# OpenRendererBenchmark/libYafaRay

Hardware: AMD Instinct MI355X
Metric: Mrays/sec (primary+secondary) on the path-tracing hot path (higher is better)
Workload: dtype f32; 1 GPU; 1M-tri diffuse Cornell-box soup 512x512 64spp primary+1-bounce (BASELINE.json metric config); triangles=1000000, width=512, height=512, spp=64, bounces=1, lights=1, parallelism=pixel-tile shard x1, film_reduce=none, kd_nodes=2803313, kd_leaf_refs=3155999, kd_max_depth=27

## Files before the change

### include/yafgpu.h

```cpp
#ifndef YAFGPU_H
#define YAFGPU_H

#include <stdint.h>

#ifdef __cplusplus
extern "C" {
#endif

#define YAFGPU_FILM_CHANNELS 5
#define YAFGPU_FILM_PLANES   4

enum { YAFGPU_MAT_SHINYDIFFUSE = 0, YAFGPU_MAT_GLOSSY = 1, YAFGPU_MAT_LIGHT = 2, YAFGPU_MAT_GLASS = 3, YAFGPU_MAT_MIRROR = 4,
       YAFGPU_MAT_COATED_GLOSSY = 5,
       YAFGPU_MAT_ROUGH_GLASS = 6,
       YAFGPU_MAT_MASKED = 7,
       YAFGPU_MAT_BLEND = 8 };
enum { YAFGPU_LIGHT_AREA = 0, YAFGPU_LIGHT_POINT = 1, YAFGPU_LIGHT_DIRECTIONAL = 2, YAFGPU_LIGHT_SUN = 3, YAFGPU_LIGHT_SPHERE = 4,
       YAFGPU_LIGHT_BACKGROUND = 5,
       YAFGPU_LIGHT_MESH = 7,
       YAFGPU_LIGHT_PORTAL = 8,
       YAFGPU_LIGHT_IES = 9, YAFGPU_LIGHT_IES_SOFT = 10,
       YAFGPU_LIGHT_SPOT = 11, YAFGPU_LIGHT_SPOT_SOFT = 12 };
enum { YAFGPU_BACKGROUND_NONE = 0, YAFGPU_BACKGROUND_CONSTANT = 1, YAFGPU_BACKGROUND_TEXTURE = 2,
       YAFGPU_BACKGROUND_GRADIENT = 4, YAFGPU_BACKGROUND_SUNSKY = 5 };
// ... 309 lines not shown
	int32_t format;
	int32_t image_width, image_height, border_x, border_y;
} yafgpu_image_desc;
uint64_t yafgpu_image_bytes(int32_t format, int32_t width, int32_t height);
int yafgpu_film_to_image(const float *d_film, const yafgpu_image_desc *desc, void *d_image, void *stream);
int yafgpu_scene_film_to_image(yafgpu_scene_t *scene, const yafgpu_image_desc *desc, void *h_image);

int yafgpu_render_passes_to_host(yafgpu_scene_t *scene, const yafgpu_render_params *rp, const yafgpu_aa_schedule *aa,
                                 float *h_film, yafgpu_counters *h_counters, int32_t *resampled);
int yafgpu_render_to_host(yafgpu_scene_t *scene, const yafgpu_render_params *rp, float *h_film, yafgpu_counters *h_counters);

int yafgpu_trace_closest(yafgpu_scene_t *scene, int32_t n, const float *rays, int32_t *tri, float *t, float *bary);
int yafgpu_trace_shadow(yafgpu_scene_t *scene, int32_t n, const float *rays, int32_t *shadowed);
uint32_t yafgpu_trace_reservation(uint32_t n, uint32_t seen, uint32_t waves);
void yafgpu_trace_schedule(uint32_t info[8]);

int yafgpu_set_profiling(yafgpu_scene_t *scene, int32_t enable);
int yafgpu_scene_set_pass_pipelining(yafgpu_scene_t *scene, int32_t mode);
void yafgpu_glibc_rand(uint32_t seed, int32_t count, int32_t *out);
int yafgpu_scene_set_abort_flag(yafgpu_scene_t *scene, const volatile int32_t *flag);
typedef int (*yafgpu_exchange_fn)(void *user, float *d_values, uint64_t n_floats);
int yafgpu_scene_set_exchange(yafgpu_scene_t *scene, yafgpu_exchange_fn fn, void *user);
int yafgpu_get_profile(const yafgpu_scene_t *scene, double ms[4], uint64_t launches[4]);

int yafgpu_probe(yafgpu_scene_t *scene, int32_t op, int32_t n, const float *in, int32_t n_in, float *out, int32_t n_out);

typedef struct yafgpu_kdtree yafgpu_kdtree_t;
yafgpu_kdtree_t *yafgpu_kdtree_build_device(const float *verts, int32_t n_tris);
yafgpu_kdtree_t *yafgpu_kdtree_build(const float *verts, int32_t n_tris, int32_t threads);
void yafgpu_kdtree_info(const yafgpu_kdtree_t *tree, yafgpu_tree_info *info);
void yafgpu_kdtree_get(const yafgpu_kdtree_t *tree, uint32_t *nodes, uint32_t *refs, float bound6[6]);
int32_t yafgpu_kdtree_treelets(const uint32_t *nodes, uint32_t n_nodes, int32_t inline_leaves, uint32_t *words, uint32_t *n_words,
                               uint32_t *leaves, uint32_t *n_leaves, uint32_t *root);
void yafgpu_kdtree_destroy(yafgpu_kdtree_t *tree);

int yafgpu_scene_get_tree(const yafgpu_scene_t *scene, uint32_t *nodes, uint32_t *refs, float bound6[6]);

#ifdef __cplusplus
}
#endif
#endif
```

### libyafaray_amd/csrc/kdtree_build.cpp

```cpp
#include "kdtree_build.h"

#include <algorithm>
#include <chrono>
#include <cmath>
#include <cstdlib>
#include <cstring>
#include <future>
#include <thread>
#include <utility>

namespace yafgpu {
namespace {

struct Box { float lo[3], hi[3]; };

struct Params
{
	const Box *prim_box;
	const float *verts;
	int depth_cap;
	float cost_ratio, empty_bonus;
};

struct Sub
// ... 326 lines not shown
		todo.emplace_back(g, (uint32_t)t);
		return (uint32_t)t << 2;
	};
	out.root = link_of(0u);
	while(!todo.empty() && !overflow)
	{
		const auto [g, t] = todo.back(); todo.pop_back();
		uint32_t w[8] = {nodes[g].a, 0u, 0u, nodes[g].b & 3u, 0u, 0u, 0u, 0u};
		const uint32_t child[2] = {g + 1u, nodes[g].b >> 2};
		uint32_t grand[4] = {0u, 0u, 0u, 0u}; bool interior[2];
		for(int k = 0; k < 2; ++k)
		{
			const KdNode &c = nodes[child[k]];
			interior[k] = (c.b & 3u) != 3u;
			w[1 + k] = interior[k] ? c.a : 0u;
			w[3] |= (interior[k] ? (c.b & 3u) : 3u) << (2 * (k + 1));
			if(interior[k]) { grand[2 * k] = child[k] + 1u; grand[2 * k + 1] = c.b >> 2; }
		}
		uint32_t links[4] = {0u, 0u, 0u, 0u};
		const size_t mark = todo.size();
		for(int k = 0; k < 2; ++k)
		{
			if(!interior[k]) { links[2 * k] = leaf_link(nodes[child[k]]); continue; }
			links[2 * k] = link_of(grand[2 * k]);
			links[2 * k + 1] = link_of(grand[2 * k + 1]);
		}
		std::reverse(todo.begin() + (std::ptrdiff_t)mark, todo.end());
		for(int k = 0; k < 4; ++k) w[4 + k] = links[k];
		std::memcpy(&out.words[(size_t)t * 8], w, sizeof w);
	}
	return overflow ? -2 : 0;
}

}

#include "../../include/yafgpu.h"
struct yafgpu_kdtree { yafgpu::KdTree t; int n_tris; };
extern "C" {
int32_t yafgpu_kdtree_treelets(const uint32_t *nodes, uint32_t n_nodes, int32_t inline_leaves, uint32_t *words, uint32_t *n_words,
                                uint32_t *leaves, uint32_t *n_leaves, uint32_t *root)
{
	std::vector<yafgpu::KdNode> tn(n_nodes);
	if(n_nodes) std::memcpy(tn.data(), nodes, (size_t)n_nodes * sizeof(yafgpu::KdNode));
	yafgpu::TreeletLayout tl;
	if(const int rc = yafgpu::build_treelets(tn, inline_leaves != 0, tl)) return rc;
	if(words && tl.words.size() <= *n_words && !tl.words.empty()) std::memcpy(words, tl.words.data(), tl.words.size() * 4);
	if(leaves && tl.leaves.size() <= *n_leaves && !tl.leaves.empty()) std::memcpy(leaves, tl.leaves.data(), tl.leaves.size() * 4);
	*n_words = (uint32_t)tl.words.size(); *n_leaves = (uint32_t)tl.leaves.size(); *root = tl.root;
	return 0;
}
yafgpu_kdtree_t *yafgpu_kdtree_build(const float *verts, int32_t n_tris, int32_t threads)
{
	auto *k = new yafgpu_kdtree();
	k->n_tris = n_tris;
	yafgpu::build_kdtree(verts, n_tris, 48, threads, k->t);
	return k;
}
void yafgpu_internal_set_error(const char *msg);
yafgpu_kdtree_t *yafgpu_kdtree_build_device(const float *verts, int32_t n_tris)
{
	auto *k = new yafgpu_kdtree();
	k->n_tris = n_tris;
	std::string err;
	if(yafgpu::build_kdtree_device_retry(verts, n_tris, 48, k->t, &err)) { yafgpu_internal_set_error(err.c_str()); delete k; return nullptr; }
	return k;
}
void yafgpu_kdtree_info(const yafgpu_kdtree_t *k, yafgpu_tree_info *info)
{
	info->n_nodes = (uint32_t)k->t.nodes.size(); info->n_leaf_refs = (uint32_t)k->t.refs.size();
	info->max_depth = (uint32_t)k->t.max_depth; info->n_tris = (uint32_t)k->n_tris;
	info->build_seconds = k->t.build_seconds; info->upload_seconds = 0; info->device_bytes = 0;
}
void yafgpu_kdtree_get(const yafgpu_kdtree_t *k, uint32_t *nodes, uint32_t *refs, float bound6[6])
{
	if(nodes && !k->t.nodes.empty()) std::memcpy(nodes, k->t.nodes.data(), k->t.nodes.size() * sizeof(yafgpu::KdNode));
	if(refs && !k->t.refs.empty()) std::memcpy(refs, k->t.refs.data(), k->t.refs.size() * sizeof(uint32_t));
	if(bound6) for(int i = 0; i < 3; ++i) { bound6[i] = k->t.bound_lo[i]; bound6[3 + i] = k->t.bound_hi[i]; }
}
void yafgpu_kdtree_destroy(yafgpu_kdtree_t *k) { delete k; }
}
```

### libyafaray_amd/csrc/kdtree_build.h

```cpp
#pragma once
#include <cstdint>
#include <string>
#include <vector>

namespace yafgpu {

struct KdNode { uint32_t a, b; };

struct KdTree
{
	std::vector<KdNode> nodes;
	std::vector<uint32_t> refs;
	float bound_lo[3], bound_hi[3];
	int max_depth = 0;
	double build_seconds = 0;
};

void build_kdtree(const float *verts, int n_tris, int depth_cap, int threads, KdTree &out);

int build_kdtree_device(const float *verts, int n_tris, int depth_cap, KdTree &out, std::string *err, int room = 1);
int build_kdtree_device_retry(const float *verts, int n_tris, int depth_cap, KdTree &out, std::string *err);

constexpr uint32_t kLinkLeaf = 0x80000000u, kLinkEscape = 0x40000000u, kLinkIndex = 0x3fffffffu, kLinkEmpty = kLinkLeaf;
constexpr uint32_t kLinkFirstBits = 24u, kLinkCountMax = 63u;
struct TreeletLayout
{
	std::vector<uint32_t> words;
	std::vector<uint32_t> leaves;
	uint32_t root = kLinkEmpty;
};
int build_treelets(const std::vector<KdNode> &nodes, bool inline_leaves, TreeletLayout &out);

}
```

### libyafaray_amd/csrc/yafgpu_device.hip

```cpp
#include <hip/hip_runtime.h>

#include <algorithm>
#include <atomic>
#include <chrono>
#include <cmath>
#include <cstdio>
#include <cstdlib>
#include <cstring>
#include <string>
#include <vector>
#include <map>
#include <memory>
#include <mutex>

#include "../../include/yafgpu.h"
#include "kdtree_build.h"
#include "yafgpu_math.h"
#include "yafgpu_shading.h"
#include "yafgpu_texture.h"
#include "yafgpu_assemble.h"

namespace yafgpu {

constexpr int kWave = 64;
constexpr int kBlock = 256;
constexpr int kWavesPerBlock = kBlock / kWave;
#ifndef YAFGPU_STACK
#define YAFGPU_STACK 8
#endif
constexpr int kStack = YAFGPU_STACK;
constexpr int kDepthCap = 48;
constexpr float kMinRayDist = (float)0.00005;
constexpr float kShadowBias = (float)0.0005;

struct DevScene
{
	const uint2 *nodes;
	const uint4 *treelets;
	const uint2 *tl_leaves;
	uint32_t tl_root;
	const uint32_t *refs;
	const float4 *tri;
	const float4 *tri_ng;
	const float4 *tri_vn;
	const yafgpu_material *mats;
	const yafgpu_light *lights;
	const int *faure;
	const int *faure_far;
	const int *faure_off;
	const double *inv_prims;
	int n_lights, n_tris, n_mats, n_faure;
	int faure_near;
	uint32_t n_nodes;
	float blo[3], bhi[3];
	yafgpu_camera cam;
	TexScene tex;
	BgScene bg;
	const float *lgeo;
};

struct RenderArgs
{
	DevScene sc;
	yafgpu_render_params rp;
	float shadow_bias, ray_min_dist, filterw;
	float table_scale; int wide_filter;
	const float *filter_table;
	int n_tiles;
	const int4 *tile_rect;
	float *planes;
	yafgpu_counters *counters;
};

struct LaneCounters { uint32_t closest, shadow, interior, leaves, tests, samples, restarts; };

// ... 832 lines not shown
	if(!bg_has_energy(row[1])) bad |= 1u << 16;
	row[kBgFlag] = __uint_as_float(bad);
}

YG_DEV void lgeo_rows(yafgpu_light *lights, int k, float *lgeo)
{
	const int n = lights[k].mesh_count;
	float *row = lgeo + lights[k].mesh_row, *func = row + kLgeoFunc;
	for(int i = (int)threadIdx.x; i < n; i += (int)blockDim.x)
	{
		const float *q = lgeo + 9 * (size_t)(lights[k].mesh_pool + i);
		const V3 a = vec3(q), edge_1 = vec3(q + 3) - a, edge_2 = vec3(q + 6) - a;
		func[i] = (float)(0.5 * (double)length(cross(edge_1, edge_2)));
	}
	__syncthreads();
	if(threadIdx.x != 0) return;
	double total_area = 0.0;
	for(int i = 0; i < n; ++i) total_area += (double)func[i];
	const float integral = pdf1d_cumulate(func, n, func + n);
	row[0] = integral; row[1] = 1.f / integral;
	lights[k].area = (float)total_area;
}
__global__ __launch_bounds__(kBlock) void meshlight_rows_kernel(yafgpu_light *lights, int n_lights, float *lgeo)
{
	const int k = (int)blockIdx.x;
	if(k >= n_lights || lights[k].type != YAFGPU_LIGHT_MESH) return;
	lgeo_rows(lights, k, lgeo);
}
__global__ __launch_bounds__(kBlock) void portallight_rows_kernel(yafgpu_light *lights, int n_lights, float *lgeo)
{
	const int k = (int)blockIdx.x;
	if(k >= n_lights || lights[k].type != YAFGPU_LIGHT_PORTAL) return;
	lgeo_rows(lights, k, lgeo);
}

}

using namespace yafgpu;

static float host_fsin(float x);
static thread_local std::string g_err;
static int fail(int code, const std::string &msg) { g_err = msg; return code; }
#define HIP_OK(expr) do { hipError_t e_ = (expr); if(e_ != hipSuccess) return fail(-100, std::string(#expr) + ": " + hipGetErrorString(e_)); } while(0)

template<typename T> struct DevMem
{
	T *p = nullptr; size_t cap = 0;
	DevMem() = default;
	DevMem(const DevMem &) = delete; DevMem &operator=(const DevMem &) = delete;
	~DevMem() { if(p) (void)hipFree(p); }
	hipError_t alloc(size_t count) { return hipMalloc((void **)&p, std::max<size_t>(count, 1) * sizeof(T)); }
	hipError_t reserve(size_t count, hipStream_t stream)
	{
		if(p && count <= cap) return hipSuccess;
		hipError_t e = hipStreamSynchronize(stream);
		if(e != hipSuccess) return e;
		if(p) (void)hipFree(p);
		p = nullptr; cap = 0;
		if((e = alloc(count)) != hipSuccess) { p = nullptr; return e; }
		cap = count;
		return hipSuccess;
	}
	operator T *() const { return p; }
};
struct Stream
{
// ... 553 lines not shown
	if(on_device)
	{
		std::string err;
		const int brc = build_kdtree_device_retry(rows.verts, n_tris, kDepthCap, s->tree, &err);
		if(brc == -2 || brc == -3) build_kdtree(rows.verts, n_tris, kDepthCap, d->build_threads, s->tree);
		else if(brc) return fail(-20, err);
	}
	else build_kdtree(rows.verts, n_tris, kDepthCap, d->build_threads, s->tree);
	s->info.build_seconds = s->tree.build_seconds;
	s->info.n_nodes = (uint32_t)s->tree.nodes.size();
	s->info.n_leaf_refs = (uint32_t)s->tree.refs.size();
	s->info.max_depth = (uint32_t)s->tree.max_depth;
	s->info.n_tris = (uint32_t)n_tris;
	return 0;
}

static int upload_tree(yafgpu_scene *s)
{
	DevScene &dv = s->dev;
	int rc = 0;
	if((rc = upload(s, (const uint2 *)s->tree.nodes.data(), s->tree.nodes.size(), &dv.nodes))) return rc;
	const char *e = std::getenv("YAFGPU_TREELET_INLINE");
	TreeletLayout tl;
	if(build_treelets(s->tree.nodes, !(e && std::atoi(e) == 0), tl)) return fail(-2, "kd-tree too large for the treelet layout");
	dv.tl_root = tl.root;
	if((rc = upload(s, (const uint4 *)tl.words.data(), tl.words.size() / 4, &dv.treelets))) return rc;
	if((rc = upload(s, (const uint2 *)tl.leaves.data(), tl.leaves.size() / 2, &dv.tl_leaves))) return rc;
	if((rc = upload(s, s->tree.refs.data(), s->tree.refs.size(), &dv.refs))) return rc;
	dv.n_nodes = (uint32_t)s->tree.nodes.size();
	for(int k = 0; k < 3; ++k) { dv.blo[k] = s->tree.bound_lo[k]; dv.bhi[k] = s->tree.bound_hi[k]; }
	return 0;
}

static int upload_lights(yafgpu_scene *s, const yafgpu_scene_desc *d)
{
	s->h_lights.assign(d->lights, d->lights + d->n_lights);
	bool with_tris = false;
	for(const yafgpu_light &l : s->h_lights) with_tris = with_tris || l.type == YAFGPU_LIGHT_MESH || l.type == YAFGPU_LIGHT_PORTAL;
	size_t row = with_tris ? (size_t)std::max(d->n_light_tris, 0) * 9 : 0;
	for(yafgpu_light &l : s->h_lights)
		if(l.type == YAFGPU_LIGHT_MESH || l.type == YAFGPU_LIGHT_PORTAL) { l.mesh_row = (int32_t)row; row += 2 * (size_t)l.mesh_count + 3; }
	row = (row + 3) & ~(size_t)3;
	for(yafgpu_light &l : s->h_lights)
		if(l.type == YAFGPU_LIGHT_PORTAL) { l.mesh_first = row <= (size_t)INT32_MAX ? (int32_t)row : 0; row += 16 * (size_t)l.mesh_count; }
	s->ies_base = row;
	for(const yafgpu_light &l : s->h_lights) s->has_ies = s->has_ies || l.type == YAFGPU_LIGHT_IES || l.type == YAFGPU_LIGHT_IES_SOFT;
	if(s->has_ies) row += (size_t)d->n_ies_floats;
	for(yafgpu_light &l : s->h_lights)
		if(l.type == YAFGPU_LIGHT_IES || l.type == YAFGPU_LIGHT_IES_SOFT) l.ies_first = row <= (size_t)INT32_MAX ? (int32_t)(s->ies_base + (size_t)l.ies_first) : 0;
	if(row > (size_t)INT32_MAX) return fail(-3, "the light-geometry pool outgrows 2^31 floats");
	s->lgeo_floats = row;
	const int rc = upload(s, s->h_lights.data(), s->h_lights.size(), &s->dev.lights);
	if(rc) return rc;
	s->dev.n_lights = s->n_lights = d->n_lights;
	for(const yafgpu_light &l : s->h_lights) s->light_mask |= 1u << (uint32_t)l.type;
	if(d->background.kind == YAFGPU_BACKGROUND_TEXTURE) s->light_mask |= 1u << (uint32_t)YAFGPU_LIGHT_BACKGROUND;
	return 0;
}

static int upload_textures(yafgpu_scene *s, const yafgpu_scene_desc *d)
{
	DevScene &dv = s->dev;
	std::memset(&dv.tex, 0, sizeof dv.tex);
	if(!((d->n_nodes > 0 && d->nodes) || d->background.kind == YAFGPU_BACKGROUND_TEXTURE)) return 0;
	int rc = 0;
	const float4 *texels = nullptr;
// ... 141 lines not shown

const char *yafgpu_last_error(void) { return g_err.c_str(); }
extern "C" void yafgpu_internal_set_error(const char *msg) { g_err = msg ? msg : ""; }

int yafgpu_device_count(void)
{
	int n = 0;
	if(hipGetDeviceCount(&n) != hipSuccess) return 0;
	return n;
}
int yafgpu_set_device(int device) { HIP_OK(hipSetDevice(device)); return 0; }

uint64_t yafgpu_planes_bytes(int32_t width, int32_t height)
{
	return (uint64_t)YAFGPU_FILM_PLANES * (uint64_t)width * (uint64_t)height * YAFGPU_FILM_CHANNELS * sizeof(float);
}

int yafgpu_scene_create(const yafgpu_scene_desc *d, yafgpu_scene_t **out)
{
	if(!out) return fail(-1, "null argument");
	int rc = check_desc(d);
	if(rc) return rc;
	std::unique_ptr<yafgpu_scene> owner(new yafgpu_scene());
	yafgpu_scene *s = owner.get();
	classify_materials(s, d);
	AssembledRows rows;
	const auto tr = std::chrono::steady_clock::now();
	if(d->inst.n_segments <= 0) host_rows(d, rows);
	else if((rc = assemble_scene(s, d, rows))) return rc;
	const double rows_seconds = std::chrono::duration<double>(std::chrono::steady_clock::now() - tr).count();
	if((rc = build_tree(s, d, rows))) return rc;
	const auto t1 = std::chrono::steady_clock::now();
	DevScene &dv = s->dev;
	if((rc = upload_tree(s)) || (rc = upload_rows(s, d, rows))) return rc;
	dv.tri = rows.rec; dv.tri_ng = rows.ng; dv.tri_vn = rows.vn; dv.mats = rows.mats;
	dv.n_tris = (int)rows.n; dv.n_mats = d->n_materials;
	if((rc = upload_lights(s, d)) || (rc = upload_textures(s, d)) || (rc = upload_nodes(s, d, rows)) || (rc = upload_qmc_tables(s))) return rc;
	dv.cam = d->camera;
	bokeh_table(dv.cam);
	s->mats.assign(d->materials, d->materials + d->n_materials);
	if((rc = background_tables(s, d)) || (rc = mesh_light_rows(s, d))) return rc;
	s->info.upload_seconds = std::chrono::duration<double>(std::chrono::steady_clock::now() - t1).count() + rows_seconds;
	*out = owner.release();
	return 0;
}

void yafgpu_scene_destroy(yafgpu_scene_t *s) { delete s; }

int yafgpu_scene_info(const yafgpu_scene_t *s, yafgpu_tree_info *info)
{
	if(!s || !info) return fail(-1, "null argument");
	*info = s->info;
	return 0;
}

int yafgpu_scene_get_tree(const yafgpu_scene_t *s, uint32_t *nodes, uint32_t *refs, float bound6[6])
{
	if(!s) return fail(-1, "null argument");
	if(nodes) std::memcpy(nodes, s->tree.nodes.data(), s->tree.nodes.size() * sizeof(KdNode));
	if(refs) std::memcpy(refs, s->tree.refs.data(), s->tree.refs.size() * sizeof(uint32_t));
	if(bound6) for(int k = 0; k < 3; ++k) { bound6[k] = s->tree.bound_lo[k]; bound6[3 + k] = s->tree.bound_hi[k]; }
	return 0;
}

static float host_fexp2(float x)
{
	x = std::min(x, 129.00000f);
// ... 1299 lines not shown
```

### libyafaray_amd/csrc/yafgpu_wavefront.h

```cpp
#pragma once

#include <stdint.h>
#if defined(__HIPCC__)
#define YAFGPU_HOST_DEVICE __host__ __device__
#else
#define YAFGPU_HOST_DEVICE
#endif
#ifndef YAFGPU_TRACE_BATCH
#define YAFGPU_TRACE_BATCH 512
#endif
#ifndef YAFGPU_TRACE_BATCH_MIN
#define YAFGPU_TRACE_BATCH_MIN 128
#endif
#ifndef YAFGPU_TRACE_BATCH_DIV
#define YAFGPU_TRACE_BATCH_DIV 8
#endif
#ifndef YAFGPU_TRACE_BATCH_SHRINK
#define YAFGPU_TRACE_BATCH_SHRINK 1
#endif
#ifndef YAFGPU_TRACE_STATIC_FIRST
#define YAFGPU_TRACE_STATIC_FIRST 1
#endif

namespace yafgpu {
// ... 2087 lines not shown
		auto leaf_end = [&]() {
			const uint2 top = stk.col[((stk.sp - 1) & (kStack - 1)) * kWave];
			const bool hit_here = !kAny && hit && z <= tmax;
			const bool emp = stk.empty();
			const bool restart = emp && stk.lost() && !(tmax >= t_exit);
			if(kStats && !YAFGPU_STATS_OCCLUDED && restart && !hit_here) ++cn.restarts;
			tmin = restart ? restart_from(tmin, tmax) : tmax;
			link = emp ? root : top.x;
			tmax = emp ? t_exit : __uint_as_float(top.y);
			stk.sp = emp ? 0 : stk.sp - 1;
			stk.lo = emp ? 0 : stk.lo;
			const bool fin = hit_here || (emp && !restart) || z < tmin;
			ws = fin ? kWalkEnd : kWalk;
		};
		auto tri_step = [&](const float4 r0, const float4 r1, const float4 r2, const uint32_t ref_v) {
			float t, u, v;
			if(kStats) ++cn.tests;
			const bool ok = tri_test_flat(r0, r1, r2, from, dir, t, u, v);
#if YAFGPU_TRACE_VIS_PIN
			uint32_t vis_w = __float_as_uint(r1.w);
			asm volatile("; visibility word of the record" : "+v"(vis_w));
			const uint32_t vis = vis_w >> 30;
#else
			const uint32_t vis = __float_as_uint(r1.w) >> 30;
#endif
			if(kAny)
			{
				const bool found = ok && t < dist && t >= ray_tmin && (vis == 0u || vis == 2u);
				hit = hit || found; done = done || found;
			}
			else
			{
				const bool better = ok && t < z && t >= ray_tmin && (vis == 0u || vis == 1u);
				z = better ? t : z; tri = better ? (int)ti : tri; bu = better ? u : bu; bv = better ? v : bv; hit = hit || better;
			}
			++p_cur; ti = ref_v;
			if(p_cur >= p_end)
			{
				if(YAFGPU_TRACE_POSTPONE)
				{
					const bool ends = !kAny && hit && z <= p_tmax;
					done = done || ends;
					if(kStats) { if(done) { cn.interior -= spec; cn.leaves -= spec_leaves; } spec = 0u; spec_leaves = 0u; }
					if(!kAny && ws != kWalkEnd && z < tmin) ws = kWalkEnd;
					ws = (ws == kBlocked) ? kWalk : ws;
				}
				else if(!done) leaf_end();
			}
		};
		auto node_step = [&](const uint4 t0, const uint4 t1) {
			const uint32_t sl = link & 3u;
			const uint32_t axis = (t0.w >> (2u * sl)) & 3u;
			const float split = __uint_as_float(sl == 0u ? t0.x : (sl == 1u ? t0.y : t0.z));
			const float2 oi = axis_col[axis * kWave];
			const float o = oi.x;
			const float tplane = (split - o) * oi.y;
			const bool dn = ((dneg >> axis) & 1u) != 0u;
#if YAFGPU_TRACE_BELOW_MASKS
			const bool below = __builtin_amdgcn_inverse_ballot_w64(__ballot(o < split) | (__ballot(o == split) & __ballot(dn)));
#else
			const bool below = dn ? (o <= split) : (o < split);
#endif
			const bool l_in = sl == 0u && ((t0.w >> 2) & 3u) != 3u, r_in = sl == 0u && ((t0.w >> 4) & 3u) != 3u;
			const uint32_t left = l_in ? (link | 1u) : (sl == 2u ? t1.z : t1.x);
			const uint32_t right = r_in ? (link | 2u) : (sl == 0u ? t1.z : (sl == 1u ? t1.y : t1.w));
			const uint32_t near_c = below ? left : right, far_c = below ? right : left;
			if(kStats) { ++cn.interior; if(p_cur < p_end) ++spec; }
			const bool near_only = !(tplane <= tmax) || tplane <= 0.f;
			const bool far_only = !near_only && tplane < tmin;
			const bool both = !near_only && !far_only;
			stk.col[(stk.sp & (kStack - 1)) * kWave] = make_uint2(far_c, __float_as_uint(tmax));
			stk.sp += both ? 1 : 0;
			stk.lo = max(stk.lo, stk.sp - (kStack - 1));
			link = far_only ? far_c : near_c;
			tmax = both ? tplane : tmax;
		};
		auto leaf_step = [&]() {
			uint32_t first = link & ((1u << kLinkFirstBits) - 1u), np = (link >> kLinkFirstBits) & kLinkCountMax;
			if(link & kLinkEscape) { const uint2 e = sc.tl_leaves[link & kLinkIndex]; first = e.x; np = e.y; }
			if(np == 0u) { if(kStats) { ++cn.leaves; if(p_cur < p_end) ++spec_leaves; } leaf_end(); }
			else if(!YAFGPU_TRACE_POSTPONE)
			{
				if(kStats) ++cn.leaves;
				p_cur = first; p_end = first + np; p_tmax = tmax; ti = sc.refs[first]; ws = kBlocked;
			}
			else if(p_cur < p_end) ws = kBlocked;
			else
			{
				if(kStats) ++cn.leaves;
				p_cur = first; p_end = first + np; p_tmax = tmax;
				ti = sc.refs[first];
				leaf_end();
			}
		};
		if(n_tri * kVoteNum >= n_node * kVoteDen && n_tri > 0)
		{
			if(kStats) ++rounds_tri;
			if(has_pend)
			{
				uint32_t ref_v = 0u;
				if(p_cur + 1u < p_end) ref_v = sc.refs[p_cur + 1u];
				const float4 r0 = sc.tri[3u * ti], r1 = sc.tri[3u * ti + 1u], r2 = sc.tri[3u * ti + 2u];
				tri_step(r0, r1, r2, ref_v);
			}
		}
		else
		{
#pragma unroll 1
			for(int s = 0; s < kNodeBurst; ++s)
			{
				if(kStats && __ballot(ws == kWalk) != 0ull) ++rounds_node;
				if(ws == kWalk && (link & kLinkLeaf)) leaf_step();
				const bool fetch = ws == kWalk && !(link & kLinkLeaf);
				const uint32_t at = link >> 2;
				uint4 t0 = make_uint4(0u, 0u, 0u, 0u), t1 = t0;
				if(fetch) { t0 = sc.treelets[2u * at]; t1 = sc.treelets[2u * at + 1u]; }
				if(fetch) node_step(t0, t1);
				if(ws == kWalk && (link & kLinkLeaf)) leaf_step();
				if(fetch && ws == kWalk && (link >> 2) == at) node_step(t0, t1);
			}
		}
		if(done || (ws == kWalkEnd && p_cur >= p_end))
		{
			if(kStats && YAFGPU_STATS_OCCLUDED && kAny && hit) ++cn.restarts;
			const bool hold = kDefer && !exhausted && (!kAny || hit);
			if(!hold) answer();
			ws = hold ? kAnswer : kNoRay; done = false; p_cur = p_end = 0u;
		}
	}
#if YAFGPU_TRACE_EXIT_LOG
	if(n != 0u)
	{
		const unsigned long long log_t1 = wall_clock64();
		if(lane == 0)
		{
// ... 445 lines not shown
```

### libyafaray_amd/interface.py

```python
import ctypes as C
import os
import sys

import numpy as np

_HERE = os.path.dirname(os.path.abspath(__file__))


def lib_path():
    return os.environ.get("YAFARAY_LIBRARY") or os.path.join(_HERE, "libyafaray_gpu.so")


class YafaRayError(RuntimeError):
    pass


class RenderStats(C.Structure):
    _fields_ = [
        ("rays_closest", C.c_uint64), ("rays_shadow", C.c_uint64), ("interior_steps", C.c_uint64), ("leaves", C.c_uint64),
        ("tri_tests", C.c_uint64), ("camera_samples", C.c_uint64), ("restarts", C.c_uint64),
        ("tree_build_seconds", C.c_double), ("upload_seconds", C.c_double), ("render_seconds", C.c_double),
        ("kd_nodes", C.c_uint32), ("kd_leaf_refs", C.c_uint32), ("kd_max_depth", C.c_uint32), ("n_triangles", C.c_uint32),
        ("scene_device_bytes", C.c_uint64),
    ]
# ... 21 lines not shown
_lib = None

C_API_SYMBOLS = [
    "yafaray_createInterface", "yafaray_destroyInterface", "yafaray_getLastError", "yafaray_getVersion",
    "yafaray_startScene", "yafaray_startGeometry", "yafaray_endGeometry", "yafaray_getNextFreeId",
    "yafaray_startTriMesh", "yafaray_endTriMesh", "yafaray_addVertex", "yafaray_addNormal", "yafaray_addTriangle",
    "yafaray_smoothMesh", "yafaray_getMeshCornerNormals", "yafaray_getLights", "yafaray_getBackground", "yafaray_getSky", "yafaray_getCamera", "yafaray_getIntegratorAO", "yafaray_getMaskMaterial", "yafaray_getIesLight", "yafaray_getBlendMaterial", "yafaray_getMaterialTable", "yafaray_addTriangles",
    "yafaray_startTriMeshPtr", "yafaray_addVertexWithOrco", "yafaray_addUv", "yafaray_addTriangleWithUv",
    "yafaray_startCurveMesh", "yafaray_endCurveMesh", "yafaray_addCurves", "yafaray_getCurves", "yafaray_addInstance", "yafaray_getInstances",
    "yafaray_paramsSetColorArray", "yafaray_paramsSetMatrix", "yafaray_paramsSetMatrixD", "yafaray_setInputColorSpace",
    "yafaray_createObject", "yafaray_createVolumeRegion", "yafaray_createImageHandler",
    "yafaray_setLoggingAndBadgeSettings", "yafaray_setupRenderPasses", "yafaray_setInteractive", "yafaray_getRenderParameters",
    "yafaray_setConsoleVerbosityLevel", "yafaray_setLogVerbosityLevel", "yafaray_setParamsBadgePosition", "yafaray_getDrawParams",
    "yafaray_printDebug", "yafaray_printVerbose", "yafaray_printInfo", "yafaray_printParams", "yafaray_printWarning", "yafaray_printError",
    "yafaray_setOutput2",
    "yafaray_paramsSetPoint", "yafaray_paramsSetString", "yafaray_paramsSetBool", "yafaray_paramsSetInt",
    "yafaray_paramsSetFloat", "yafaray_paramsSetColor", "yafaray_paramsClearAll", "yafaray_paramsStartList",
    "yafaray_paramsPushList", "yafaray_paramsEndList",
    "yafaray_createTexture", "yafaray_createTextureFromMemory", "yafaray_getTextureImage",
    "yafaray_createLight", "yafaray_createMaterial", "yafaray_createCamera", "yafaray_createBackground",
    "yafaray_createIntegrator", "yafaray_clearAll", "yafaray_render", "yafaray_abort", "yafaray_getRenderedImage",
    "yafaray_getFilm", "yafaray_getRenderStats", "yafaray_setShard", "yafaray_setPlaneExchange", "yafaray_setSerialReplay", "yafaray_getRandState", "yafaray_setRandState", "yafaray_prepareRender",
    "yafaray_renderPassDevice", "yafaray_getRenderSize", "yafaray_loadXml", "yafaray_intersectRays", "yafaray_shadowRays", "yafaray_probe", "yafaray_setProfiling", "yafaray_getKernelProfile", "yafaray_setPassPipelining",
    "yafaray_commGetUniqueId", "yafaray_commCreate", "yafaray_commDestroy", "yafaray_commRank", "yafaray_commWorld", "yafaray_commLastError",
    "yafaray_commBackend", "yafaray_reduceFilm", "yafaray_allReduce", "yafaray_commExchange", "yafaray_setComm",
    "yafaray_setFilmPath", "yafaray_getFilmPath", "yafaray_getFilmResume", "yafaray_writeFilmFile", "yafaray_readFilmFile", "yafaray_filmLastError",
    "yafaray_createImageOutput", "yafaray_destroyImageOutput", "yafaray_imageOutputLastError", "yafaray_imageOutputCallbacks",
    "yafaray_filmToImage", "yafaray_writeImageFile",
]
GPU_ABI_SYMBOLS = [
    "yafgpu_last_error", "yafgpu_device_count", "yafgpu_set_device", "yafgpu_scene_create", "yafgpu_scene_destroy",
    "yafgpu_scene_info", "yafgpu_planes_bytes", "yafgpu_render_tiles", "yafgpu_film_combine", "yafgpu_render_to_host", "yafgpu_render_passes_to_host",
    "yafgpu_trace_closest", "yafgpu_trace_shadow", "yafgpu_trace_reservation", "yafgpu_trace_schedule", "yafgpu_scene_get_tree", "yafgpu_probe",
    "yafgpu_kdtree_build", "yafgpu_kdtree_build_device", "yafgpu_kdtree_info", "yafgpu_kdtree_get", "yafgpu_kdtree_destroy", "yafgpu_kdtree_treelets",
    "yafgpu_set_profiling", "yafgpu_scene_set_pass_pipelining", "yafgpu_get_profile", "yafgpu_scene_set_abort_flag", "yafgpu_scene_set_exchange", "yafgpu_glibc_rand",
    "yafgpu_image_bytes", "yafgpu_film_to_image", "yafgpu_scene_film_to_image",
]


def load():
    global _lib
    if _lib is not None:
        return _lib
    p = lib_path()
    if not os.path.exists(p):
        raise YafaRayError(f"{p} not found: build it with `python -c 'import __graft_entry__ as g; g.build()'` "
                           f"(libyafaray_amd/csrc/build.sh); there is no CPU fallback")
    L = C.CDLL(p)
    vp, cp, ci, cd, cf = C.c_void_p, C.c_char_p, C.c_int, C.c_double, C.c_float
    sig = {
        "yafaray_createInterface": (vp, []), "yafaray_destroyInterface": (None, [vp]),
        "yafaray_getLastError": (cp, [vp]), "yafaray_getVersion": (cp, []),
        "yafaray_startScene": (ci, [vp, ci]), "yafaray_startGeometry": (ci, [vp]), "yafaray_endGeometry": (ci, [vp]),
        "yafaray_getNextFreeId": (C.c_uint, [vp]),
        "yafaray_startTriMesh": (ci, [vp, C.c_uint, ci, ci, ci, ci, ci, ci]), "yafaray_endTriMesh": (ci, [vp]),
        "yafaray_addVertex": (ci, [vp, cd, cd, cd]), "yafaray_addNormal": (None, [vp, cd, cd, cd]),
        "yafaray_addTriangle": (ci, [vp, ci, ci, ci, vp]), "yafaray_smoothMesh": (ci, [vp, C.c_uint, cd]),
        "yafaray_getMeshCornerNormals": (ci, [vp, C.c_uint, C.POINTER(cf), ci]),
        "yafaray_getLights": (ci, [vp, vp, ci]),
        "yafaray_getBackground": (ci, [vp, cp, vp]),
        "yafaray_getSky": (ci, [vp, cp, vp]),
        "yafaray_getCamera": (ci, [vp, cp, vp]),
        "yafaray_getIntegratorAO": (ci, [vp, cp, C.POINTER(ci), C.POINTER(ci), C.POINTER(cf), C.POINTER(cf)]),
        "yafaray_getMaskMaterial": (ci, [vp, cp, vp]),
        "yafaray_getBlendMaterial": (ci, [vp, cp, vp]),
        "yafaray_getIesLight": (ci, [vp, cp, C.POINTER(ci), C.POINTER(ci), C.POINTER(ci), C.POINTER(cf), C.POINTER(cf), C.POINTER(cf), ci]),
        "yafaray_getMaterialTable": (ci, [vp, vp, ci]),
# ... 636 lines not shown
        if not h:
            raise YafaRayError("device kd build: " + L.yafgpu_last_error().decode())
    else:
        h = L.yafgpu_kdtree_build(v.ctypes.data_as(C.POINTER(C.c_float)), v.shape[0], threads)
    info = TreeInfo()
    L.yafgpu_kdtree_info(h, C.byref(info))
    nodes = np.zeros((max(info.n_nodes, 1), 2), np.uint32)
    refs = np.zeros(max(info.n_leaf_refs, 1), np.uint32)
    bound = np.zeros(6, np.float32)
    up = C.POINTER(C.c_uint32)
    L.yafgpu_kdtree_get(h, nodes.ctypes.data_as(up), refs.ctypes.data_as(up), bound.ctypes.data_as(C.POINTER(C.c_float)))
    L.yafgpu_kdtree_destroy(h)
    return nodes[:info.n_nodes], refs[:info.n_leaf_refs], bound, info


def build_treelets(nodes, inline_leaves=True):
    L = load()
    up = C.POINTER(C.c_uint32)
    L.yafgpu_kdtree_treelets.argtypes = [up, C.c_uint32, C.c_int32, up, up, up, up, up]
    nd = np.ascontiguousarray(nodes, dtype=np.uint32).reshape(-1, 2)
    nw, nl, root = C.c_uint32(0), C.c_uint32(0), C.c_uint32(0)
    rc = L.yafgpu_kdtree_treelets(nd.ctypes.data_as(up), nd.shape[0], int(bool(inline_leaves)), None, C.byref(nw), None, C.byref(nl), C.byref(root))
    if rc:
        raise YafaRayError(f"treelet layout: {rc}")
    words = np.zeros(max(nw.value, 1), np.uint32)
    leaves = np.zeros(max(nl.value, 1), np.uint32)
    rc = L.yafgpu_kdtree_treelets(nd.ctypes.data_as(up), nd.shape[0], int(bool(inline_leaves)), words.ctypes.data_as(up), C.byref(nw),
                                  leaves.ctypes.data_as(up), C.byref(nl), C.byref(root))
    if rc:
        raise YafaRayError(f"treelet layout: {rc}")
    return words[:nw.value].reshape(-1, 8), leaves[:nl.value].reshape(-1, 2), root.value


def trace_reservation(n, seen, waves):
    L = load()
    L.yafgpu_trace_reservation.argtypes = [C.c_uint32, C.c_uint32, C.c_uint32]
    L.yafgpu_trace_reservation.restype = C.c_uint32
    return int(L.yafgpu_trace_reservation(n, seen, waves))


def trace_schedule():
    L = load()
    info = (C.c_uint32 * 8)()
    L.yafgpu_trace_schedule.argtypes = [C.POINTER(C.c_uint32)]
    L.yafgpu_trace_schedule.restype = None
    L.yafgpu_trace_schedule(info)
    keys = ("min", "max", "div", "shrink", "static_first", "waves_per_group", "grid_closest", "grid_any")
    return dict(zip(keys, (int(v) for v in info)))


def planes_bytes(width, height):
    return load().yafgpu_planes_bytes(width, height)


def film_combine(d_planes, d_film, width, height, stream=0):
    rc = load().yafgpu_film_combine(C.c_void_p(d_planes), C.c_void_p(d_film), width, height, C.c_void_p(stream or None))
    if rc:
        raise YafaRayError(load().yafgpu_last_error().decode())


FILM_HEADER_FIELDS = tuple(k for k, _ in FilmHeader._fields_)


def film_last_error():
    return load().yafaray_filmLastError().decode()

# ... 35 lines not shown
```

Measured before the change: 2954 Mrays/s.

## Reorder triangle records into kd-tree leaf traversal order for cache locality

At scene upload, triangles are renumbered by first appearance in the kd-tree leaf reference list. A reordered copy of the triangle records is built on device with the original id kept in the w lane of the third record, and the leaf refs are remapped to the new positions. The traversal loop reads from these walk copies and recovers the original triangle id from r2.w for the hit. The aim is more coherent memory access during leaf intersection, at the cost of extra device memory for the duplicated triangle and ref arrays plus a small upload-time kernel.

```diff
diff --git a/include/yafgpu.h b/include/yafgpu.h
--- a/include/yafgpu.h
+++ b/include/yafgpu.h
@@ -365,6 +365,7 @@
 void yafgpu_kdtree_get(const yafgpu_kdtree_t *tree, uint32_t *nodes, uint32_t *refs, float bound6[6]);
 int32_t yafgpu_kdtree_treelets(const uint32_t *nodes, uint32_t n_nodes, int32_t inline_leaves, uint32_t *words, uint32_t *n_words,
                                uint32_t *leaves, uint32_t *n_leaves, uint32_t *root);
+void yafgpu_kdtree_tri_order(const uint32_t *refs, uint32_t n_refs, uint32_t n_tris, uint32_t *pos);
 void yafgpu_kdtree_destroy(yafgpu_kdtree_t *tree);
 
 int yafgpu_scene_get_tree(const yafgpu_scene_t *scene, uint32_t *nodes, uint32_t *refs, float bound6[6]);
diff --git a/libyafaray_amd/csrc/kdtree_build.cpp b/libyafaray_amd/csrc/kdtree_build.cpp
--- a/libyafaray_amd/csrc/kdtree_build.cpp
+++ b/libyafaray_amd/csrc/kdtree_build.cpp
@@ -382,6 +382,19 @@
 	return overflow ? -2 : 0;
 }
 
+void tri_order(const uint32_t *refs, size_t n_refs, uint32_t n_tris, std::vector<uint32_t> &pos)
+{
+	constexpr uint32_t kNone = 0xffffffffu;
+	pos.assign((size_t)n_tris, kNone);
+	uint32_t rank = 0u;
+	for(size_t i = 0; i < n_refs; ++i)
+	{
+		const uint32_t t = refs[i];
+		if(t < n_tris && pos[t] == kNone) pos[t] = rank++;
+	}
+	for(uint32_t t = 0u; t < n_tris; ++t) if(pos[t] == kNone) pos[t] = rank++;
+}
+
 }
 
 #include "../../include/yafgpu.h"
@@ -427,5 +440,11 @@
 	if(refs && !k->t.refs.empty()) std::memcpy(refs, k->t.refs.data(), k->t.refs.size() * sizeof(uint32_t));
 	if(bound6) for(int i = 0; i < 3; ++i) { bound6[i] = k->t.bound_lo[i]; bound6[3 + i] = k->t.bound_hi[i]; }
 }
+void yafgpu_kdtree_tri_order(const uint32_t *refs, uint32_t n_refs, uint32_t n_tris, uint32_t *pos)
+{
+	std::vector<uint32_t> p;
+	yafgpu::tri_order(refs, (size_t)n_refs, n_tris, p);
+	if(pos && !p.empty()) std::memcpy(pos, p.data(), p.size() * sizeof(uint32_t));
+}
 void yafgpu_kdtree_destroy(yafgpu_kdtree_t *k) { delete k; }
 }
diff --git a/libyafaray_amd/csrc/kdtree_build.h b/libyafaray_amd/csrc/kdtree_build.h
--- a/libyafaray_amd/csrc/kdtree_build.h
+++ b/libyafaray_amd/csrc/kdtree_build.h
@@ -31,4 +31,6 @@
 };
 int build_treelets(const std::vector<KdNode> &nodes, bool inline_leaves, TreeletLayout &out);
 
+void tri_order(const uint32_t *refs, size_t n_refs, uint32_t n_tris, std::vector<uint32_t> &pos);
+
 }
diff --git a/libyafaray_amd/csrc/yafgpu_device.hip b/libyafaray_amd/csrc/yafgpu_device.hip
--- a/libyafaray_amd/csrc/yafgpu_device.hip
+++ b/libyafaray_amd/csrc/yafgpu_device.hip
@@ -41,6 +41,8 @@
 	uint32_t tl_root;
 	const uint32_t *refs;
 	const float4 *tri;
+	const float4 *tri_walk;
+	const uint32_t *refs_walk;
 	const float4 *tri_ng;
 	const float4 *tri_vn;
 	const yafgpu_material *mats;
@@ -939,6 +941,26 @@
 	const int k = (int)blockIdx.x;
 	if(k >= n_lights || lights[k].type != YAFGPU_LIGHT_PORTAL) return;
 	lgeo_rows(lights, k, lgeo);
+}
+
+__global__ __launch_bounds__(kBlock) void walk_copy_kernel(const float4 *rec, const uint32_t *pos, uint32_t n_tris, const uint32_t *refs, uint32_t n_refs,
+                                                            float4 *tri_walk, uint32_t *refs_walk)
+{
+	const size_t stride = (size_t)gridDim.x * blockDim.x, i0 = (size_t)blockIdx.x * blockDim.x + threadIdx.x;
+	for(size_t t = i0; t < (size_t)n_tris; t += stride)
+	{
+		const size_t p = pos[t];
+		if(p >= (size_t)n_tris) continue;
+		const float4 r2 = rec[3 * t + 2];
+		tri_walk[3 * p] = rec[3 * t];
+		tri_walk[3 * p + 1] = rec[3 * t + 1];
+		tri_walk[3 * p + 2] = make_float4(r2.x, r2.y, r2.z, __uint_as_float((uint32_t)t));
+	}
+	for(size_t i = i0; i < (size_t)n_refs; i += stride)
+	{
+		const uint32_t t = refs[i];
+		refs_walk[i] = t < n_tris ? pos[t] : 0u;
+	}
 }
 
 }
@@ -1558,6 +1580,29 @@
 	return 0;
 }
 
+static int upload_walk_copy(yafgpu_scene *s, const AssembledRows &rows)
+{
+	DevScene &dv = s->dev;
+	const uint32_t n = rows.n, n_refs = (uint32_t)s->tree.refs.size();
+	std::vector<uint32_t> pos;
+	const char *e = std::getenv("YAFGPU_TRI_ORDER");
+	if(e && std::strcmp(e, "id") == 0) { pos.resize(n); for(uint32_t t = 0u; t < n; ++t) pos[t] = t; }
+	else tri_order(s->tree.refs.data(), s->tree.refs.size(), n, pos);
+	DevMem<uint32_t> d_pos;
+	float4 *tri_walk = nullptr; uint32_t *refs_walk = nullptr;
+	int rc = 0;
+	if((rc = temp_upload(d_pos, pos.data(), pos.size())) || (rc = scene_alloc(s, 3 * (size_t)n, &tri_walk)) || (rc = scene_alloc(s, (size_t)n_refs, &refs_walk))) return rc;
+	if(n)
+	{
+		const uint32_t blocks = std::min<uint32_t>((std::max(n, n_refs) + (uint32_t)kBlock - 1u) / (uint32_t)kBlock, 8192u);
+		hipLaunchKernelGGL(walk_copy_kernel, dim3(blocks), dim3(kBlock), 0, nullptr, rows.rec, (const uint32_t *)d_pos.p, n, dv.refs, n_refs, tri_walk, refs_walk);
+		HIP_OK(hipGetLastError());
+		HIP_OK(hipDeviceSynchronize());
+	}
+	dv.tri_walk = tri_walk; dv.refs_walk = refs_walk;
+	return 0;
+}
+
 static int upload_lights(yafgpu_scene *s, const yafgpu_scene_desc *d)
 {
 	s->h_lights.assign(d->lights, d->lights + d->n_lights);
@@ -1765,7 +1810,7 @@
 	if((rc = build_tree(s, d, rows))) return rc;
 	const auto t1 = std::chrono::steady_clock::now();
 	DevScene &dv = s->dev;
-	if((rc = upload_tree(s)) || (rc = upload_rows(s, d, rows))) return rc;
+	if((rc = upload_tree(s)) || (rc = upload_rows(s, d, rows)) || (rc = upload_walk_copy(s, rows))) return rc;
 	dv.tri = rows.rec; dv.tri_ng = rows.ng; dv.tri_vn = rows.vn; dv.mats = rows.mats;
 	dv.n_tris = (int)rows.n; dv.n_mats = d->n_materials;
 	if((rc = upload_lights(s, d)) || (rc = upload_textures(s, d)) || (rc = upload_nodes(s, d, rows)) || (rc = upload_qmc_tables(s))) return rc;
diff --git a/libyafaray_amd/csrc/yafgpu_wavefront.h b/libyafaray_amd/csrc/yafgpu_wavefront.h
--- a/libyafaray_amd/csrc/yafgpu_wavefront.h
+++ b/libyafaray_amd/csrc/yafgpu_wavefront.h
@@ -2143,7 +2143,7 @@
 			else
 			{
 				const bool better = ok && t < z && t >= ray_tmin && (vis == 0u || vis == 1u);
-				z = better ? t : z; tri = better ? (int)ti : tri; bu = better ? u : bu; bv = better ? v : bv; hit = hit || better;
+				z = better ? t : z; tri = better ? (int)__float_as_uint(r2.w) : tri; bu = better ? u : bu; bv = better ? v : bv; hit = hit || better;
 			}
 			++p_cur; ti = ref_v;
 			if(p_cur >= p_end)
@@ -2193,14 +2193,14 @@
 			else if(!YAFGPU_TRACE_POSTPONE)
 			{
 				if(kStats) ++cn.leaves;
-				p_cur = first; p_end = first + np; p_tmax = tmax; ti = sc.refs[first]; ws = kBlocked;
+				p_cur = first; p_end = first + np; p_tmax = tmax; ti = sc.refs_walk[first]; ws = kBlocked;
 			}
 			else if(p_cur < p_end) ws = kBlocked;
 			else
 			{
 				if(kStats) ++cn.leaves;
 				p_cur = first; p_end = first + np; p_tmax = tmax;
-				ti = sc.refs[first];
+				ti = sc.refs_walk[first];
 				leaf_end();
 			}
 		};
@@ -2210,8 +2210,8 @@
 			if(has_pend)
 			{
 				uint32_t ref_v = 0u;
-				if(p_cur + 1u < p_end) ref_v = sc.refs[p_cur + 1u];
-				const float4 r0 = sc.tri[3u * ti], r1 = sc.tri[3u * ti + 1u], r2 = sc.tri[3u * ti + 2u];
+				if(p_cur + 1u < p_end) ref_v = sc.refs_walk[p_cur + 1u];
+				const float4 r0 = sc.tri_walk[3u * ti], r1 = sc.tri_walk[3u * ti + 1u], r2 = sc.tri_walk[3u * ti + 2u];
 				tri_step(r0, r1, r2, ref_v);
 			}
 		}
diff --git a/libyafaray_amd/interface.py b/libyafaray_amd/interface.py
--- a/libyafaray_amd/interface.py
+++ b/libyafaray_amd/interface.py
@@ -77,7 +77,7 @@
     "yafgpu_last_error", "yafgpu_device_count", "yafgpu_set_device", "yafgpu_scene_create", "yafgpu_scene_destroy",
     "yafgpu_scene_info", "yafgpu_planes_bytes", "yafgpu_render_tiles", "yafgpu_film_combine", "yafgpu_render_to_host", "yafgpu_render_passes_to_host",
     "yafgpu_trace_closest", "yafgpu_trace_shadow", "yafgpu_trace_reservation", "yafgpu_trace_schedule", "yafgpu_scene_get_tree", "yafgpu_probe",
-    "yafgpu_kdtree_build", "yafgpu_kdtree_build_device", "yafgpu_kdtree_info", "yafgpu_kdtree_get", "yafgpu_kdtree_destroy", "yafgpu_kdtree_treelets",
+    "yafgpu_kdtree_build", "yafgpu_kdtree_build_device", "yafgpu_kdtree_info", "yafgpu_kdtree_get", "yafgpu_kdtree_destroy", "yafgpu_kdtree_treelets", "yafgpu_kdtree_tri_order",
     "yafgpu_set_profiling", "yafgpu_scene_set_pass_pipelining", "yafgpu_get_profile", "yafgpu_scene_set_abort_flag", "yafgpu_scene_set_exchange", "yafgpu_glibc_rand",
     "yafgpu_image_bytes", "yafgpu_film_to_image", "yafgpu_scene_film_to_image",
 ]
@@ -780,6 +780,17 @@
     return words[:nw.value].reshape(-1, 8), leaves[:nl.value].reshape(-1, 2), root.value
 
 
+def tri_order(refs, n_tris):
+    L = load()
+    up = C.POINTER(C.c_uint32)
+    L.yafgpu_kdtree_tri_order.argtypes = [up, C.c_uint32, C.c_uint32, up]
+    L.yafgpu_kdtree_tri_order.restype = None
+    r = np.ascontiguousarray(refs, dtype=np.uint32).reshape(-1)
+    pos = np.zeros(max(int(n_tris), 1), np.uint32)
+    L.yafgpu_kdtree_tri_order(r.ctypes.data_as(up), r.shape[0], int(n_tris), pos.ctypes.data_as(up))
+    return pos[:int(n_tris)]
+
+
 def trace_reservation(n, seen, waves):
     L = load()
     L.yafgpu_trace_reservation.argtypes = [C.c_uint32, C.c_uint32, C.c_uint32]
```

Measured after the change: 3056 Mrays/s, median of 6. +3.4%, better.
